# Polochon-street/bliss-rs

Measured on AMD Instinct MI355X. Metric: songs/sec (3-min 22 050 Hz f32) at 1/2/4/8 GPU; HBM GB/s vs roofline, higher is better.
Workload: dtype f32; 1 GPU; configs[1]: batch of 1024 synthetic 3969000-sample (3-min) white-noise f32 PCM buffers per GPU, full 23-feature descriptor set (FeaturesVersion 2); songs_per_gpu=1024, songs_total=1024, features=23, parallelism=single GPU

## Files before the change

### bliss-rs_amd/csrc/kernels_chroma.hip

```cpp
#include <float.h>
#include <stdlib.h>

#include <type_traits>

#include "device_utils.hpp"
#include "fft_r16.hpp"
#include "internal.hpp"

namespace bg {

typedef double double4_t __attribute__((ext_vector_type(4)));

__device__ __forceinline__ double tuning_of_slot(int slot) {
    return slot >= N_TUNING ? 0.0 : (-50.0 + (100.0 * 0.01 * (double)slot)) / 100.0;
}

__global__ __launch_bounds__(256) void chroma_bank_kernel(double* __restrict__ bank) {
#pragma clang fp contract(off)
    const int slot = blockIdx.y;
    const int k = blockIdx.x * 256 + threadIdx.x;
    if (k >= BANK_PITCH) return;
    double* out = bank + (size_t)slot * BANK_ROWS * BANK_PITCH;
    if (k >= CBINS) {
        for (int r = 0; r < BANK_ROWS; r++) out[(size_t)r * BANK_PITCH + k] = 0.0;
// ... 441 lines not shown
        const float thr = ref_floor_f32(ref);
        {
            uint32_t hits = 0;
#pragma unroll
            for (int h = 0; h < 2; h++) {
                float sb3[3], se3[3], sa3[3];
#pragma unroll
                for (int q = 0; q < 3; q++) {
                    const int c = t + 256 * (3 * h + q);
                    sb3[q] = mags[c > 0 ? c - 1 : 0];
                    se3[q] = mags[c];
                    sa3[q] = mags[c + 1];
                }
#pragma unroll
                for (int q = 0; q < 3; q++) {
                    const int j = 3 * h + q, c = t + 256 * j;
                    const uint32_t in_range = (256 * j >= PIP_LO && 256 * j + 255 <= PIP_HI) ? 1u : (uint32_t)(c >= PIP_LO) & (uint32_t)(c <= PIP_HI);
                    const uint32_t pk = in_range & (uint32_t)(sa3[q] <= se3[q]) & (uint32_t)(sb3[q] < se3[q]) & (uint32_t)(se3[q] > thr);
                    hits |= pk << j;
                }
            }
            const uint32_t mine = (uint32_t)__popc(hits);
            const uint32_t incl = wave_scan_incl_u32_dpp(mine);
            uint32_t wbase = 0;
            if (lane_id() == 63) wbase = atomicAdd(&peak_count, incl);
            uint32_t pos = (uint32_t)__builtin_amdgcn_readlane((int)wbase, 63) + incl - mine;
#pragma unroll
            for (int j = 0; j < 6; j++)
                if ((hits >> j) & 1u) peak_list[pos++] = (uint16_t)(t + 256 * j);
            TRACE(13);
            __syncthreads();
            TRACE(14);
            const uint32_t n_peaks = peak_count;
            uint32_t* __restrict__ recs = peak_rec + (sd.c_off + f) * (size_t)PIP_MAX_PER_FRAME;
            if (t == 0) peak_cnt[sd.c_off + f] = n_peaks;
            int c_next = t < n_peaks ? (int)peak_list[t] : PIP_LO;
            for (uint32_t i = t; i < n_peaks; i += 256) {
                const int c = c_next;
                const float sb = mags[c - 1], se = mags[c], sa = mags[c + 1];
                c_next = i + 256 < n_peaks ? (int)peak_list[i + 256] : PIP_LO;
                int pb;
                const uint32_t b = peak_classify(sb, se, sa, ref, c, &pb), rel = b - lbase;
                recs[i] = peak_record(b, pb, c);
                if (rel < (uint32_t)LHIST_BINS) atomicAdd(&lhist[rel], 1u);
                else atomicAdd(&hist[b], 1u);
            }
        }
        __builtin_amdgcn_s_setprio(0);
        if (has_next) {
            load_window();
#pragma unroll
            for (int n1 = 0; n1 < 16; n1++) v[n1] = v[n1] * win[n1];
        }
        TRACE(15);
        __syncthreads();
        TRACE(16);
    }
    TRACE_FLUSH();
    if (have_base) {
        const uint32_t lbase = lhist_base;
        for (int i = t; i < LHIST_BINS; i += 256) {
            const uint32_t c = lhist[i];
            if (c) atomicAdd(&hist[lbase + i], c);
        }
    }
}

void launch_stft8192(const Batch& b, const Workspace& w, const DeviceTables& t, hipStream_t st, int shape) {
    if (b.tiles_c == 0) return;
    auto k = stft8192_kernel<false, false>;
    if (shape == 1) k = stft8192_kernel<true, true>;
    else if (shape == 2) k = stft8192_kernel<true, false>;
    else if (shape == 3) k = stft8192_kernel<false, true>;
    hipLaunchKernelGGL(k, dim3((b.tiles_c + 31u) & ~31u), dim3(256), 0, st,
                       b.pcm, b.songs, b.n_songs, b.pfx_c, t.hann8192, t.tw8192, w.spec, w.frame_max, w.h1, w.peak_rec, w.peak_cnt,
                       b.tiles_c);
}

__global__ __launch_bounds__(256) void tune_select_kernel(const SongDesc* __restrict__ songs,
                                                          const uint32_t* __restrict__ h1,
                                                          TuningState* __restrict__ tuning,
                                                          uint32_t* __restrict__ cand_cursor, uint32_t cand_pool,
                                                          uint32_t first_song) {
    __shared__ uint32_t wsum[4];
    __shared__ uint32_t s_total, s_blo, s_bhi;
    const uint32_t s = blockIdx.x + first_song;
    const int tid = threadIdx.x;
    TuningState* ts = tuning + s;
    auto no_peaks = [&]() {
        if (tid == 0) {
            ts->n_peaks = 0; ts->tuning_idx = -1; ts->n_cand = 0; ts->b_lo = 1; ts->b_hi = 0; ts->below = 0;
            ts->cand_off = 0; ts->cand_cap = 0;
        }
    };
    if (!songs[s].ok) { no_peaks(); return; }
    const uint32_t* hist = h1 + (size_t)s * H1_BINS;
    constexpr int PER = H1_BINS / 256;
    uint32_t local[PER], sum = 0;
#pragma unroll
    for (int i = 0; i < PER; i++) { local[i] = hist[tid * PER + i]; sum += local[i]; }
    const uint32_t incl = wave_scan_incl_u32(sum);
    if (lane_id() == 63) wsum[wave_id()] = incl;
    __syncthreads();
    uint32_t base = 0;
    for (int w = 0; w < wave_id(); w++) base += wsum[w];
    if (tid == 255) s_total = base + incl;
    __syncthreads();
    const uint32_t total = s_total;
    uint32_t before = base + incl - sum;
    if (total == 0) { no_peaks(); return; }
    const uint32_t r_lo = (total - 1) / 2, r_hi = total - 1 - r_lo;
    if (tid == 0) { ts->n_peaks = total; ts->n_cand = 0; ts->tuning_idx = -1; }
#pragma unroll
    for (int i = 0; i < PER; i++) {
        const uint32_t c = local[i];
        if (c) {
            if (before <= r_lo && r_lo < before + c) { ts->b_lo = tid * PER + i; ts->below = before; s_blo = tid * PER + i; }
            if (before <= r_hi && r_hi < before + c) { ts->b_hi = tid * PER + i; s_bhi = tid * PER + i; }
        }
        before += c;
    }
    __syncthreads();
    const uint32_t blo = s_blo, bhi = s_bhi;
    uint32_t mine = 0;
#pragma unroll
    for (int i = 0; i < PER; i++) {
        const uint32_t bin = tid * PER + i;
        if (bin >= blo && bin <= bhi) mine += local[i];
    }
    mine = wave_sum(mine);
    if (lane_id() == 0) wsum[wave_id()] = mine;
    __syncthreads();
    if (tid == 0) {
        const uint32_t want = wsum[0] + wsum[1] + wsum[2] + wsum[3];
        const uint32_t off = atomicAdd(cand_cursor, want);
        if (off <= cand_pool && want <= cand_pool - off) {
            ts->cand_off = off;
            ts->cand_cap = want;
        } else {
            atomicSub(cand_cursor, want);
            ts->cand_off = 0;
            ts->cand_cap = 0;
        }
    }
}

void launch_tune_select(const Batch& b, const Workspace& w, hipStream_t st, const SongRange* r) {
    const uint32_t s0 = r ? r->s0 : 0, s1 = r ? r->s1 : b.n_songs;
    if (s1 <= s0) return;
    hipLaunchKernelGGL(tune_select_kernel, dim3(s1 - s0), dim3(256), 0, st, b.songs, w.h1, w.tuning, w.cand_cursor,
                       w.cand_cap, s0);
}

constexpr int P2_SLOW_CAP = 1024;
constexpr int P2_FRAMES_PER_WAVE = CH_TILE / 4;

__global__ __launch_bounds__(256) void tune_pass2_kernel(const SongDesc* __restrict__ songs, uint32_t n_songs,
                                                         const uint32_t* __restrict__ pfx_ct,
                                                         const float* __restrict__ spec,
                                                         const float* __restrict__ frame_max,
                                                         const uint32_t* __restrict__ peak_rec,
                                                         const uint32_t* __restrict__ peak_cnt,
                                                         TuningState* __restrict__ tuning,
                                                         uint32_t* __restrict__ hist100,
                                                         double* __restrict__ cand_mag,
                                                         uint8_t* __restrict__ cand_pb, uint32_t first_tile) {
    __shared__ uint32_t hist[N_TUNING];
    __shared__ uint32_t slow_list[4][P2_SLOW_CAP];
    const uint32_t bx = blockIdx.x + first_tile;
    const uint32_t s = find_segment(pfx_ct, n_songs, bx);
    const SongDesc sd = songs[s];
    const uint32_t tile = bx - pfx_ct[s];
    const int tid = threadIdx.x, lane = lane_id(), wave = wave_id();
    TuningState* ts = tuning + s;
    const uint32_t b_lo = ts->b_lo, b_hi = ts->b_hi;
    if (ts->n_peaks == 0) return;
    const uint32_t cand_off = ts->cand_off;
    const uint32_t cand_cap = ts->cand_cap;
    const bool pooled = cand_cap != 0;
    if (tid < N_TUNING) hist[tid] = 0;
    __syncthreads();
    uint32_t n_slow = 0;

    auto flush = [&]() {
        for (uint32_t i = lane; i < n_slow; i += WAVE) {
            const uint32_t e = slow_list[wave][i];
            const int c = (int)(e & 0xFFFFu);
            const uint32_t f = tile * CH_TILE + wave + 4 * (e >> 16);
            const float* row = spec + (sd.c_off + f) * (size_t)CBINS_PAD;
            const double ref = 0.1 * (double)frame_max[sd.c_off + f];
            double mag, pitch;
            if (pip_peak_core(row[c - 1], row[c], row[c + 1], ref, c, &mag, &pitch)) {
                const uint32_t b = coarse_bin(mag);
                if (b > b_hi) {
                    atomicAdd(&hist[pitch_bin(pitch)], 1u);
                } else if (b >= b_lo) {
                    const uint32_t slot = atomicAdd(&ts->n_cand, 1u);
                    if (pooled && slot < cand_cap) {
                        cand_mag[cand_off + slot] = mag;
                        cand_pb[cand_off + slot] = (uint8_t)pitch_bin(pitch);
                    }
                }
            }
        }
        __builtin_amdgcn_wave_barrier();
        n_slow = 0;
    };
    uint32_t n_rec_next = 0;
    {
        const uint32_t f0 = tile * CH_TILE + wave;
        if (f0 < sd.n_c) n_rec_next = peak_cnt[sd.c_off + f0];
    }
    for (int i = 0; i < P2_FRAMES_PER_WAVE; i++) {
        const uint32_t f = tile * CH_TILE + wave + 4 * i;
        if (f >= sd.n_c) break;
        const uint32_t n_rec = n_rec_next < (uint32_t)PIP_MAX_PER_FRAME ? n_rec_next : (uint32_t)PIP_MAX_PER_FRAME;
        if (i + 1 < P2_FRAMES_PER_WAVE && f + 4 < sd.n_c) n_rec_next = peak_cnt[sd.c_off + f + 4];
        const uint32_t* __restrict__ recs = peak_rec + (sd.c_off + f) * (size_t)PIP_MAX_PER_FRAME;
        if (n_slow + PIP_MAX_PER_FRAME > P2_SLOW_CAP) flush();
        for (uint32_t j0 = 0; j0 < n_rec; j0 += 4 * WAVE) {
            uint32_t r4[4];
#pragma unroll
            for (int u = 0; u < 4; u++) {
                const uint32_t j = j0 + WAVE * u + lane;
                r4[u] = j < n_rec ? recs[j] : 0xFFFFFFFFu;
            }
#pragma unroll
            for (int u = 0; u < 4; u++) {
                if (j0 + WAVE * u >= n_rec) break;
                const uint32_t j = j0 + WAVE * u + lane;
                bool slow = false;
                uint32_t c = 0;
                if (j < n_rec) {
                    const uint32_t r = r4[u];
                    const uint32_t b = r >> 18, pbf = (r >> 11) & 0x7Fu;
                    c = r & 0x7FFu;
                    if (b > b_hi) {
                        if (pbf) atomicAdd(&hist[pbf - 1], 1u);
                        else slow = true;
                    } else if (b >= b_lo) {
                        slow = true;
                    }
                }
                const uint64_t mask = __ballot(slow);
                if (mask) {
                    if (slow) slow_list[wave][n_slow + (uint32_t)__popcll(mask & ((1ull << lane) - 1ull))] = ((uint32_t)i << 16) | c;
                    n_slow += (uint32_t)__popcll(mask);
                }
            }
        }
    }
    __builtin_amdgcn_wave_barrier();
    flush();
    __syncthreads();
    if (tid < N_TUNING && hist[tid]) atomicAdd(&hist100[(size_t)s * N_TUNING + tid], hist[tid]);
}

void launch_tune_pass2(const Batch& b, const Workspace& w, hipStream_t st, const SongRange* r) {
    const uint32_t t0 = r ? r->ct0 : 0, t1 = r ? r->ct1 : b.tiles_ct;
    if (t1 <= t0) return;
    hipLaunchKernelGGL(tune_pass2_kernel, dim3(t1 - t0), dim3(256), 0, st, b.songs, b.n_songs, b.pfx_ct, w.spec,
                       w.frame_max, w.peak_rec, w.peak_cnt, w.tuning, w.hist100, w.cand_mag, w.cand_pb, t0);
}

template <typename ForEach>
__device__ uint64_t block_radix_select(ForEach&& for_each, uint32_t rank, uint32_t* hist, uint32_t* s_digit, uint32_t* s_rank,
                                       uint32_t* s_wave) {
    const int tid = threadIdx.x;
    uint64_t prefix = 0, mask = 0;
    for (int shift = 56; shift >= 0; shift -= 8) {
        hist[tid] = 0;
        __syncthreads();
        for_each([&](double mag, int) {
            const uint64_t k = f64_key(mag);
            const bool in = (k & mask) == prefix;
            const uint32_t d = (uint32_t)(k >> shift) & 0xFFu;
            const uint64_t m = __ballot(in);
            if (m != 0) {
                const int first = __ffsll((unsigned long long)m) - 1;
                const uint32_t d0 = (uint32_t)__shfl((int)d, first, WAVE);
                if (__ballot(in && d == d0) == m) {
                    if (lane_id() == first) atomicAdd(&hist[d0], (uint32_t)__popcll(m));
                } else if (in) {
                    atomicAdd(&hist[d], 1u);
                }
            }
        });
        __syncthreads();
        {
            const uint32_t h = hist[tid];
            const uint32_t incl = wave_scan_incl_u32(h);
            if (lane_id() == 63) s_wave[wave_id()] = incl;
            __syncthreads();
            uint32_t below = incl - h;
            for (int w = 0; w < wave_id(); w++) below += s_wave[w];
            if (h != 0 && below <= rank && rank < below + h) {
                *s_digit = (uint32_t)tid;
                *s_rank = rank - below;
            }
        }
        __syncthreads();
        prefix |= (uint64_t)(*s_digit) << shift;
        mask |= 0xFFull << shift;
        rank = *s_rank;
        __syncthreads();
    }
    return prefix;
}

__global__ __launch_bounds__(256) void tune_final_kernel(const SongDesc* __restrict__ songs,
                                                         TuningState* __restrict__ tuning,
                                                         const uint32_t* __restrict__ hist100,
                                                         const double* __restrict__ cand_mag,
                                                         const uint8_t* __restrict__ cand_pb,
                                                         const float* __restrict__ spec,
                                                         const float* __restrict__ frame_max,
                                                         const uint32_t* __restrict__ peak_rec,
                                                         const uint32_t* __restrict__ peak_cnt, uint32_t first_song) {
    __shared__ uint32_t hist[256];
    __shared__ uint32_t s_digit, s_rank, s_cnt_le, s_wave[4];
    __shared__ unsigned long long s_min_gt;
    const uint32_t s = blockIdx.x + first_song;
    const int tid = threadIdx.x;
    TuningState* ts = tuning + s;
    const SongDesc sd = songs[s];
    if (!sd.ok || ts->n_peaks == 0) return;
    const uint32_t total = ts->n_peaks, nc = ts->n_cand;
    const uint32_t r_lo = (total - 1) / 2, r_hi = total - 1 - r_lo;
    const uint32_t k_lo = r_lo - ts->below, k_hi = r_hi - ts->below;
    const uint32_t b_lo = ts->b_lo, b_hi = ts->b_hi;
    const bool pooled = ts->cand_cap != 0 && nc == ts->cand_cap;
    const double* v = cand_mag + ts->cand_off;
    const uint8_t* pb = cand_pb + ts->cand_off;

    auto for_each = [&](auto&& fn) {
        if (pooled) {
            for (uint32_t i0 = tid; i0 < nc; i0 += 8 * 256) {
                double m8[8];
                int b8[8];
#pragma unroll
                for (int u = 0; u < 8; u++) {
                    const uint32_t i = i0 + 256u * u;
                    m8[u] = i < nc ? v[i] : 0.0;
                    b8[u] = i < nc ? (int)pb[i] : 0;
                }
#pragma unroll
                for (int u = 0; u < 8; u++)
                    if (i0 + 256u * u < nc) fn(m8[u], b8[u]);
            }
        } else {
            for (uint32_t f = 0; f < sd.n_c; f++) {
                const uint32_t n_rec_raw = peak_cnt[sd.c_off + f];
                const uint32_t n_rec = n_rec_raw < (uint32_t)PIP_MAX_PER_FRAME ? n_rec_raw : (uint32_t)PIP_MAX_PER_FRAME;
                const uint32_t* __restrict__ recs = peak_rec + (sd.c_off + f) * (size_t)PIP_MAX_PER_FRAME;
                const float* __restrict__ row = spec + (sd.c_off + f) * (size_t)CBINS_PAD;
                const double ref = 0.1 * (double)frame_max[sd.c_off + f];
                for (uint32_t j = tid; j < n_rec; j += 256) {
                    const uint32_t r = recs[j], b = r >> 18;
                    if (b < b_lo || b > b_hi) continue;
                    const int c = (int)(r & 0x7FFu);
                    double mag, pitch;
                    if (pip_peak_core(row[c - 1], row[c], row[c + 1], ref, c, &mag, &pitch)) fn(mag, pitch_bin(pitch));
                }
            }
        }
    };

    const uint64_t key_lo = block_radix_select(for_each, k_lo, hist, &s_digit, &s_rank, s_wave);
    uint64_t key_hi = key_lo;
    if (k_hi != k_lo) {
        if (tid == 0) { s_cnt_le = 0; s_min_gt = ~0ull; }
        __syncthreads();
        uint32_t cnt = 0;
        unsigned long long mn = ~0ull;
        for_each([&](double mag, int) {
            const uint64_t k = f64_key(mag);
            if (k <= key_lo) cnt++;
            else if (k < mn) mn = k;
        });
        atomicAdd(&s_cnt_le, cnt);
        atomicMin(&s_min_gt, mn);
        __syncthreads();
        if (s_cnt_le <= k_hi) key_hi = s_min_gt;
    }
    double thr;
    {
#pragma clang fp contract(off)
        const double lo = key_f64(key_lo), hi = key_f64(key_hi);
        thr = lo + (hi - lo) / 2.0;
    }
    __syncthreads();
    if (tid < N_TUNING) hist[tid] = hist100[(size_t)s * N_TUNING + tid];
    __syncthreads();
    for_each([&](double mag, int bin) {
        if (mag >= thr) atomicAdd(&hist[bin], 1u);
    });
    __syncthreads();
    if (tid == 0) {
        uint32_t best = 0;
        for (uint32_t k = 1; k < N_TUNING; k++)
            if (hist[k] > hist[best]) best = k;
        ts->tuning_idx = (int32_t)best;
    }
}

void launch_tune_final(const Batch& b, const Workspace& w, hipStream_t st, const SongRange* r) {
// ... 161 lines not shown
```

### bliss-rs_amd/csrc/scheduler.hip

```cpp
#include <string.h>

#include <algorithm>
#include <chrono>
#include <condition_variable>
#include <numeric>

#include "coalescing_front.hpp"
#include "ctx.hpp"

using namespace bg;

namespace {

inline size_t align_up(size_t x, size_t a) { return (x + a - 1) / a * a; }

void fill_counts(SongDesc& d) {
    const uint64_t n = d.n;
    d.n_t = (uint32_t)((n - W512) / HOP_T + 1);
    d.n_b = (uint32_t)((n - W512) / HOP_B + 1);
    d.n_f = std::max(d.n_t, 2u * d.n_b);
    d.n_c = (uint32_t)ceilf((float)n / (float)HOP_C);
    d.n_e = (uint32_t)((n + 255) / 256);
    d.n_l = (uint32_t)((n + LOUD_W - 1) / LOUD_W);
}

size_t song_ws_bytes(const SongDesc& d) {
    if (!d.ok) return 256;
    size_t b = 0;
    b += (size_t)d.n_t * 12 + (size_t)d.n_b * 8 + (size_t)d.n_e * 8;
    b += (size_t)d.n_c * (CBINS_PAD * 4 + 4);
    b += (size_t)H1_BINS * 4 + N_TUNING * 4 + sizeof(TuningState) + sizeof(TempoState);
    b += (size_t)d.n_c * CAND_BUDGET_PER_FRAME * 9;
    b += (size_t)d.n_c * (PIP_MAX_PER_FRAME * 4 + 4);
    b += ((size_t)d.n_c / CH_TILE + 1) * 80;
    b += ((size_t)d.n_b / BT_STEP + 2) * (8 + BT_PRE_STRIDE * 4);
    return b + 4096;
}

struct Carver {
    uint8_t* base;
    size_t off = 0;
    template <typename T>
    T* take(size_t n) {
        off = align_up(off, 256);
        T* p = reinterpret_cast<T*>(base + off);
        off += n * sizeof(T);
        return p;
    }
};

struct ChunkTotals {
    uint64_t tot_t = 0, tot_b = 0, tot_c = 0, tot_e = 0;
    uint32_t max_nb = 0, max_nt = 0, max_runs = 1;
    uint32_t tiles_ct = 0;
    uint64_t cand_cap = 0;
};

Workspace carve(uint8_t* base, uint32_t ns, const ChunkTotals& t, size_t* bytes) {
    Carver m{base};
    Workspace w{};
    w.centroid = m.take<float>(t.tot_t); w.rolloff = m.take<float>(t.tot_t); w.flatness = m.take<float>(t.tot_t);
    w.flux = m.take<float>(t.tot_b); w.thresholded = m.take<float>(t.tot_b);
    w.e256 = m.take<float>(t.tot_e); w.zc256 = m.take<uint32_t>(t.tot_e);
    static_assert((size_t)(CBINS_PAD + PIP_MAX_PER_FRAME) * 4 * HOP_T >= (size_t)256 * 4 * HOP_C,
                  "the borrowed stretch must hold one 256-word entry per timbral frame: bytes per chroma frame x samples per "
                  "timbral frame >= bytes per entry x samples per chroma frame");
    w.spec = m.take<float>(t.tot_c * CBINS_PAD + 64);
    w.peak_rec = m.take<uint32_t>(t.tot_c * PIP_MAX_PER_FRAME);
    w.roll_fix_bytes = (size_t)(reinterpret_cast<uint8_t*>(w.peak_rec + t.tot_c * PIP_MAX_PER_FRAME) - reinterpret_cast<uint8_t*>(w.spec));
    w.frame_max = m.take<float>(t.tot_c);
    w.roll_fix = m.take<RollFix>(1);
    w.h1 = m.take<uint32_t>((size_t)ns * H1_BINS); w.hist100 = m.take<uint32_t>((size_t)ns * N_TUNING);
    w.tuning = m.take<TuningState>(ns);
    w.peak_cnt = m.take<uint32_t>(t.tot_c);
    w.cand_mag = m.take<double>(t.cand_cap); w.cand_pb = m.take<uint8_t>(t.cand_cap);
    w.cand_cursor = m.take<uint32_t>(4);
    w.cand_cap = (uint32_t)t.cand_cap;
    w.chroma_part = m.take<double>((size_t)t.tiles_ct * 10 + 16);
    w.tempo = m.take<TempoState>(ns);
    w.run_bpm = m.take<float>((size_t)ns * t.max_runs); w.run_cnt = m.take<uint32_t>((size_t)ns * t.max_runs);
    w.runs_pitch = t.max_runs;
    w.bt_pre = m.take<float>((size_t)(t.tot_b / BT_STEP + ns + 1) * BT_PRE_STRIDE);
    w.summary = m.take<float>((size_t)ns * 16);
    *bytes = m.off + 4096;
    return w;
}

int ensure_mask_stream(blissgpu_ctx* c, int cus) {
    cus = std::max(1, std::min(cus, c->n_cus));
    if (c->mask_stream && c->mask_cus == cus) return BLISSGPU_OK;
    if (c->mask_stream) { (void)hipStreamSynchronize(c->mask_stream); (void)hipStreamDestroy(c->mask_stream); c->mask_stream = nullptr; }
    std::vector<uint32_t> mask((size_t)(c->n_cus + 31) / 32, 0u);
    for (int i = 0; i < cus; i++) mask[(size_t)i / 32] |= 1u << (i % 32);
    HIP_TRY(hipExtStreamCreateWithCUMask(&c->mask_stream, (uint32_t)mask.size(), mask.data()));
    c->mask_cus = cus;
    return BLISSGPU_OK;
}

int ensure_slot_events(ChunkSlot& s) {
    if (s.ev_free) return BLISSGPU_OK;
    hipEvent_t* evs[] = {&s.ev_start, &s.ev_fork, &s.ev_stft, &s.ev_sel, &s.ev_tune, &s.ev_sum, &s.ev_chroma, &s.ev_desc, &s.ev_free, &s.ev_acf, &s.ev_beat};
    for (hipEvent_t* e : evs) HIP_TRY(hipEventCreateWithFlags(e, hipEventDisableTiming));
    for (hipEvent_t& e : s.ev_piece) HIP_TRY(hipEventCreateWithFlags(&e, hipEventDisableTiming));
    return BLISSGPU_OK;
}

int chunk_front(blissgpu_ctx* c, ChunkSlot& slot, const float* d_pcm, SongDesc* songs, uint32_t ns, bool only_chunk) {
    int rc = ensure_slot_events(slot);
    if (rc) return rc;
    std::vector<uint32_t> pfx_f(ns + 1, 0), pfx_c(ns + 1, 0), pfx_ct(ns + 1, 0), pfx_cw(ns + 1, 0);
    ChunkTotals t;
    for (uint32_t i = 0; i < ns; i++) {
        SongDesc& d = songs[i];
        d.t_off = t.tot_t; d.b_off = t.tot_b; d.c_off = t.tot_c; d.e_off = t.tot_e;
        if (d.ok) {
            t.tot_t += d.n_t; t.tot_b += d.n_b; t.tot_c += d.n_c; t.tot_e += d.n_e;
            t.max_nb = std::max(t.max_nb, d.n_b);
            t.max_nt = std::max(t.max_nt, d.n_t);
            t.max_runs = std::max(t.max_runs, d.n_b / BT_STEP + 1);
        }
        pfx_f[i + 1] = pfx_f[i] + (d.ok ? (d.n_f + F512_TILE - 1) / F512_TILE : 0);
        pfx_c[i + 1] = pfx_c[i] + (d.ok ? 4 * ((d.n_c + 4 * STFT_TILE - 1) / (4 * STFT_TILE)) : 0);
        pfx_ct[i + 1] = pfx_ct[i] + (d.ok ? (d.n_c + CH_TILE - 1) / CH_TILE : 0);
        pfx_cw[i + 1] = pfx_cw[i] + (d.ok ? (d.n_c + 4 * CH_TILE - 1) / (4 * CH_TILE) : 0);
    }
    t.tiles_ct = pfx_ct[ns];
    t.cand_cap = std::min<uint64_t>(t.tot_c * (uint64_t)c->cand_budget, 0xFFFFFF00ull) + 64;

    const size_t desc_bytes = align_up(ns * sizeof(SongDesc), 256) + 4 * align_up((ns + 1) * 4, 256) + 256;
    size_t need = 0;
    (void)carve(nullptr, ns, t, &need);
    if ((rc = slot.desc.ensure(desc_bytes))) return rc;
    if ((rc = slot.slab.ensure(need))) return rc;
    if (slot.used) HIP_TRY(hipEventSynchronize(slot.ev_desc));
    if ((rc = slot.h_desc.ensure(desc_bytes))) return rc;

    hipStream_t st = c->stream, sb = c->serial ? c->stream : c->aux_stream, sc = c->serial ? c->stream : c->chr_stream;
    const bool multi = !c->serial;
    if (slot.used && multi) HIP_TRY(hipStreamWaitEvent(st, slot.ev_free, 0));

    uint8_t* h = slot.h_desc.p;
    size_t o = 0;
    const size_t o_songs = o; memcpy(h + o, songs, ns * sizeof(SongDesc)); o = align_up(o + ns * sizeof(SongDesc), 256);
    const size_t o_f = o; memcpy(h + o, pfx_f.data(), (ns + 1) * 4); o = align_up(o + (ns + 1) * 4, 256);
    const size_t o_c = o; memcpy(h + o, pfx_c.data(), (ns + 1) * 4); o = align_up(o + (ns + 1) * 4, 256);
    const size_t o_ct = o; memcpy(h + o, pfx_ct.data(), (ns + 1) * 4); o = align_up(o + (ns + 1) * 4, 256);
    const size_t o_cw = o; memcpy(h + o, pfx_cw.data(), (ns + 1) * 4); o = align_up(o + (ns + 1) * 4, 256);
    HIP_TRY(hipMemcpyAsync(slot.desc.p, h, o, hipMemcpyHostToDevice, st));
    slot.used = true;

    Batch& b = slot.batch;
    b = Batch{};
    b.pcm = d_pcm;
    b.songs = reinterpret_cast<const SongDesc*>(slot.desc.p + o_songs);
    b.n_songs = ns;
    b.pfx_f = reinterpret_cast<const uint32_t*>(slot.desc.p + o_f);
    b.pfx_c = reinterpret_cast<const uint32_t*>(slot.desc.p + o_c);
    b.pfx_ct = reinterpret_cast<const uint32_t*>(slot.desc.p + o_ct);
    b.pfx_cw = reinterpret_cast<const uint32_t*>(slot.desc.p + o_cw);
    b.tiles_f = pfx_f[ns]; b.tiles_c = pfx_c[ns]; b.tiles_ct = pfx_ct[ns]; b.tiles_cw = pfx_cw[ns];
    b.total_b = t.tot_b; b.max_nb = t.max_nb; b.max_nt = t.max_nt;

    size_t used_bytes = 0;
    slot.ws = carve(slot.slab.p, ns, t, &used_bytes);
    slot.ws.dbg_chroma = nullptr;
    slot.ws.dbg_interval = nullptr;
    if (c->debug_chroma) {
        if ((rc = c->dbg_chroma.ensure((size_t)t.tot_c * 12 + 12))) return rc;
        if ((rc = c->dbg_interval.ensure((size_t)ns * 10))) return rc;
        slot.ws.dbg_chroma = c->dbg_chroma.p;
        slot.ws.dbg_interval = c->dbg_interval.p;
    }
    const Workspace& w = slot.ws;
    c->last_ws = w;
    c->last_songs.assign(songs, songs + ns);
    {
        RollFix rf{};
        if ((uint64_t)w.roll_fix_bytes / (256 * 4) < t.tot_t)
            return fail(BLISSGPU_ERR_INVALID, "chunk_front", "internal: the borrowed stretch cannot hold one exact-rolloff entry per timbral frame");
        rf.cap = (uint32_t)t.tot_t;
        rf.mags = w.spec;
        memcpy(h + o, &rf, sizeof(rf));
        HIP_TRY(hipMemcpyAsync(w.roll_fix, h + o, sizeof(rf), hipMemcpyHostToDevice, st));
    }
    HIP_TRY(hipEventRecord(slot.ev_desc, st));

    HIP_TRY(hipMemsetAsync(w.h1, 0, (size_t)ns * H1_BINS * 4, st));
    HIP_TRY(hipMemsetAsync(w.hist100, 0, (size_t)ns * N_TUNING * 4, st));
    HIP_TRY(hipMemsetAsync(w.cand_cursor, 0, 16, st));
    { Prof p(c, K_FFT512); launch_fft512(b, w, c->tables, st, c->rolloff_exact_all, c->flux_order); }
    { Prof p(c, K_ROLLFIX); launch_rolloff_fix(b, w, t.tot_t, st); }
    if (multi) {
        HIP_TRY(hipEventRecord(slot.ev_fork, st));
        HIP_TRY(hipStreamWaitEvent(sb, slot.ev_fork, 0));
    }
    { Prof p(c, K_ONSET, sb); launch_onset(b, w, sb); }
    { Prof p(c, K_SUMMARY, sb); launch_summary(b, w, sb); }
    slot.beat_masked = multi && c->tail_mode >= 2;
    if (slot.beat_masked) {
        if ((rc = ensure_mask_stream(c, c->tail_mode))) return rc;
        { Prof p(c, K_BEAT, sb); launch_beat_acf(b, w, c->tables, sb); }
        HIP_TRY(hipEventRecord(slot.ev_acf, sb));
        HIP_TRY(hipStreamWaitEvent(c->mask_stream, slot.ev_acf, 0));
        { Prof p(c, K_BEAT, c->mask_stream); launch_beat_track(b, w, c->tables, c->mask_stream); }
        HIP_TRY(hipEventRecord(slot.ev_beat, c->mask_stream));
    }
    const bool acf_early = multi && c->tail_mode == -2;
    if (acf_early) { Prof p(c, K_BEAT, sb); launch_beat_acf(b, w, c->tables, sb); }
    const bool beat_last = multi && c->tail_mode == -3;
    const bool beat_late = !slot.beat_masked && !beat_last && (c->tail_mode == 1 || acf_early || (c->tail_mode < 0 && only_chunk));
    if (!beat_late && !slot.beat_masked && !beat_last) { Prof p(c, K_BEAT, sb); launch_beat(b, w, c->tables, sb); }
    { Prof p(c, K_STFT8192); launch_stft8192(b, w, c->tables, st, c->stft_shape); }
    if (multi) {
        HIP_TRY(hipEventRecord(slot.ev_stft, st));
        HIP_TRY(hipStreamWaitEvent(sc, slot.ev_stft, 0));
    }
    slot.pieces = 0;
    if (multi && only_chunk && c->tail_split > 1 && ns >= 2) {
        const int want = std::min<int>(std::min<int>(c->tail_split, ChunkSlot::MAX_PIECES), (int)ns);
        uint32_t s0 = 0;
        for (int k = 0; k < want && s0 < ns; k++) {
            uint32_t s1 = s0 + 1;
            const uint64_t goal = (uint64_t)pfx_ct[ns] * (uint64_t)(k + 1) / (uint64_t)want;
            while (s1 < ns && (k == want - 1 || pfx_ct[s1] < goal)) s1++;
            slot.piece[slot.pieces++] = SongRange{s0, s1, pfx_ct[s0], pfx_ct[s1], pfx_cw[s0], pfx_cw[s1]};
            s0 = s1;
        }
        if (slot.pieces < 2) slot.pieces = 0;
    }
    if (slot.pieces) {
        for (int k = 0; k < slot.pieces; k++) {
            { Prof p(c, K_TUNE_SELECT, sc); launch_tune_select(b, w, sc, &slot.piece[k]); }
            if (k == 1 && beat_late) {
                HIP_TRY(hipEventRecord(slot.ev_sel, sc));
                HIP_TRY(hipStreamWaitEvent(sb, slot.ev_sel, 0));
                Prof p(c, K_BEAT, sb);
                if (acf_early) launch_beat_track(b, w, c->tables, sb); else launch_beat(b, w, c->tables, sb);
            }
            { Prof p(c, K_TUNE_PASS2, sc); launch_tune_pass2(b, w, sc, &slot.piece[k]); }
            { Prof p(c, K_TUNE_FINAL, sc); launch_tune_final(b, w, sc, &slot.piece[k]); }
            HIP_TRY(hipEventRecord(slot.ev_piece[k], sc));
        }
        if (beat_last) {
            HIP_TRY(hipStreamWaitEvent(sb, slot.ev_piece[slot.pieces - 1], 0));
            Prof p(c, K_BEAT, sb);
            launch_beat(b, w, c->tables, sb);
        }
        HIP_TRY(hipGetLastError());
        slot.back_pending = true;
        return BLISSGPU_OK;
    }
    { Prof p(c, K_TUNE_SELECT, sc); launch_tune_select(b, w, sc); }
    if (beat_late) {
        if (multi) {
            HIP_TRY(hipEventRecord(slot.ev_sel, sc));
            HIP_TRY(hipStreamWaitEvent(sb, slot.ev_sel, 0));
        }
        Prof p(c, K_BEAT, sb);
        if (acf_early) launch_beat_track(b, w, c->tables, sb); else launch_beat(b, w, c->tables, sb);
    }
    { Prof p(c, K_TUNE_PASS2, sc); launch_tune_pass2(b, w, sc); }
    { Prof p(c, K_TUNE_FINAL, sc); launch_tune_final(b, w, sc); }
    if (multi) HIP_TRY(hipEventRecord(slot.ev_tune, sc));
    if (beat_last) {
        HIP_TRY(hipStreamWaitEvent(sb, slot.ev_tune, 0));
        Prof p(c, K_BEAT, sb);
        launch_beat(b, w, c->tables, sb);
    }
    HIP_TRY(hipGetLastError());
    slot.back_pending = true;
    return BLISSGPU_OK;
}

int chunk_back(blissgpu_ctx* c, ChunkSlot& slot, uint32_t features_version, float* d_out, int32_t* d_status) {
    if (!slot.back_pending) return BLISSGPU_OK;
    slot.back_pending = false;
    hipStream_t st = c->stream, sb = c->serial ? c->stream : c->aux_stream;
    const bool multi = !c->serial;
    if (slot.pieces) {
        for (int k = 0; k < slot.pieces; k++) {
            HIP_TRY(hipStreamWaitEvent(st, slot.ev_piece[k], 0));
            Prof p(c, K_CHROMA);
            launch_chroma(slot.batch, slot.ws, c->tables, st, &slot.piece[k]);
        }
    } else {
        if (multi) HIP_TRY(hipStreamWaitEvent(st, slot.ev_tune, 0));
        Prof p(c, K_CHROMA);
        launch_chroma(slot.batch, slot.ws, c->tables, st);
    }
    if (multi) {
        HIP_TRY(hipEventRecord(slot.ev_chroma, st));
        HIP_TRY(hipStreamWaitEvent(sb, slot.ev_chroma, 0));
        if (slot.beat_masked) HIP_TRY(hipStreamWaitEvent(sb, slot.ev_beat, 0));
    }
    { Prof p(c, K_FINALIZE, sb); launch_finalize(slot.batch, slot.ws, features_version, d_out, d_status, c->dbg_tuning.p, c->dbg_nbpms.p, sb); }
    if (multi) HIP_TRY(hipEventRecord(slot.ev_free, sb));
    HIP_TRY(hipGetLastError());
    return BLISSGPU_OK;
}

}

namespace bg {

void scheduler_release(blissgpu_ctx* c) {
    for (ChunkSlot& s : c->slot) {
        s.slab.release(); s.desc.release(); s.h_desc.release();
        hipEvent_t evs[] = {s.ev_start, s.ev_fork, s.ev_stft, s.ev_sel, s.ev_tune, s.ev_sum, s.ev_chroma, s.ev_desc, s.ev_free, s.ev_acf, s.ev_beat};
        for (hipEvent_t e : evs)
            if (e) (void)hipEventDestroy(e);
        for (hipEvent_t e : s.ev_piece)
            if (e) (void)hipEventDestroy(e);
        s = ChunkSlot{};
    }
    HostFeed& f = c->feed;
    f.ring.reset();
    for (hipStream_t& ls : f.lane_stream)
        if (ls) { (void)hipStreamSynchronize(ls); (void)hipStreamDestroy(ls); ls = nullptr; }
    for (auto& row : f.ev_lane)
        for (hipEvent_t& ev : row)
            if (ev) { (void)hipEventDestroy(ev); ev = nullptr; }
    for (auto& kv : c->swr_banks)
        if (kv.second.d_bank) (void)hipFree(kv.second.d_bank);
    c->swr_banks.clear();
    c->swr_bytes = 0;
    for (hipStream_t& cs : f.copy_stream)
        if (cs) { (void)hipStreamSynchronize(cs); (void)hipStreamDestroy(cs); cs = nullptr; }
    for (int b = 0; b < N_FEED_BUFFERS; b++) {
        f.pcm[b].release(); f.raw[b].release(); f.out[b].release();
        for (hipEvent_t& ev : f.ev_copied[b])
            if (ev) { (void)hipEventDestroy(ev); ev = nullptr; }
        if (f.ev_done[b]) (void)hipEventDestroy(f.ev_done[b]);
        f.ev_done[b] = nullptr;
    }
}

#ifndef FEED_GROUP_MIB
// ... 656 lines not shown
```

Measured before the change: 27690 songs/sec.

## Software-pipeline tuning pass-2 record loads and batch slow-path flush gathers

Restructures tune_pass2_kernel so that each wave prefetches the next frame's peak records while it classifies the current one, and reads all per-frame counts with a single lane-parallel load plus readlane. Slow-path entries are compacted with a DPP wave scan over per-lane bitmasks instead of one ballot per word. The flush loop now issues four gathers of spectrum and frame_max per lane before it computes anything. Separately, the slow list grows to 2000 entries with launch bounds set for five workgroups per CU. The host also folds the RollFix record into the single descriptor memcpy, dropping one small H2D copy. The costs are more registers and LDS per workgroup, and a workspace pointer that now lives in the descriptor buffer.

Measured after the change: 27770 songs/sec, median of 6. Within noise of the previous version (+0.3%).

```diff
diff --git a/bliss-rs_amd/csrc/kernels_chroma.hip b/bliss-rs_amd/csrc/kernels_chroma.hip
--- a/bliss-rs_amd/csrc/kernels_chroma.hip
+++ b/bliss-rs_amd/csrc/kernels_chroma.hip
@@ -617,21 +617,26 @@
                        w.cand_cap, s0);
 }
 
-constexpr int P2_SLOW_CAP = 1024;
+constexpr int P2_SLOW_CAP = 2000;
 constexpr int P2_FRAMES_PER_WAVE = CH_TILE / 4;
-
-__global__ __launch_bounds__(256) void tune_pass2_kernel(const SongDesc* __restrict__ songs, uint32_t n_songs,
-                                                         const uint32_t* __restrict__ pfx_ct,
-                                                         const float* __restrict__ spec,
-                                                         const float* __restrict__ frame_max,
-                                                         const uint32_t* __restrict__ peak_rec,
-                                                         const uint32_t* __restrict__ peak_cnt,
-                                                         TuningState* __restrict__ tuning,
-                                                         uint32_t* __restrict__ hist100,
-                                                         double* __restrict__ cand_mag,
-                                                         uint8_t* __restrict__ cand_pb, uint32_t first_tile) {
+constexpr int P2_FLUSH = 4;
+constexpr int P2_WORDS = (PIP_MAX_PER_FRAME + WAVE - 1) / WAVE;
+static_assert(P2_WORDS <= 16 && P2_FRAMES_PER_WAVE <= WAVE, "a lane keeps one bit per record and one frame count per wave slot");
+
+__global__ __launch_bounds__(256, 5) void tune_pass2_kernel(const SongDesc* __restrict__ songs, uint32_t n_songs,
+                                                            const uint32_t* __restrict__ pfx_ct,
+                                                            const float* __restrict__ spec,
+                                                            const float* __restrict__ frame_max,
+                                                            const uint32_t* __restrict__ peak_rec,
+                                                            const uint32_t* __restrict__ peak_cnt,
+                                                            TuningState* __restrict__ tuning,
+                                                            uint32_t* __restrict__ hist100,
+                                                            double* __restrict__ cand_mag,
+                                                            uint8_t* __restrict__ cand_pb, uint32_t first_tile) {
     __shared__ uint32_t hist[N_TUNING];
     __shared__ uint32_t slow_list[4][P2_SLOW_CAP];
+    static_assert(5 * sizeof(uint32_t) * (4 * P2_SLOW_CAP + N_TUNING) <= 160 * 1024 && 6 * sizeof(uint32_t) * (4 * P2_SLOW_CAP + N_TUNING) > 160 * 1024,
+                  "exactly five workgroups fit a CU's 160 KiB of LDS");
     const uint32_t bx = blockIdx.x + first_tile;
     const uint32_t s = find_segment(pfx_ct, n_songs, bx);
     const SongDesc sd = songs[s];
@@ -648,22 +653,34 @@
     uint32_t n_slow = 0;
 
     auto flush = [&]() {
-        for (uint32_t i = lane; i < n_slow; i += WAVE) {
-            const uint32_t e = slow_list[wave][i];
-            const int c = (int)(e & 0xFFFFu);
-            const uint32_t f = tile * CH_TILE + wave + 4 * (e >> 16);
-            const float* row = spec + (sd.c_off + f) * (size_t)CBINS_PAD;
-            const double ref = 0.1 * (double)frame_max[sd.c_off + f];
-            double mag, pitch;
-            if (pip_peak_core(row[c - 1], row[c], row[c + 1], ref, c, &mag, &pitch)) {
-                const uint32_t b = coarse_bin(mag);
-                if (b > b_hi) {
-                    atomicAdd(&hist[pitch_bin(pitch)], 1u);
-                } else if (b >= b_lo) {
-                    const uint32_t slot = atomicAdd(&ts->n_cand, 1u);
-                    if (pooled && slot < cand_cap) {
-                        cand_mag[cand_off + slot] = mag;
-                        cand_pb[cand_off + slot] = (uint8_t)pitch_bin(pitch);
+        for (uint32_t i0 = 0; i0 < n_slow; i0 += P2_FLUSH * WAVE) {
+            int cc[P2_FLUSH];
+            float sb[P2_FLUSH], se[P2_FLUSH], sa[P2_FLUSH], fm[P2_FLUSH];
+#pragma unroll
+            for (int u = 0; u < P2_FLUSH; u++) {
+                const uint32_t i = i0 + (uint32_t)(WAVE * u + lane);
+                const uint32_t e = slow_list[wave][i < n_slow ? i : 0u];
+                const size_t fr = sd.c_off + tile * CH_TILE + wave + 4 * (e >> 16);
+                const int c = (int)(e & 0xFFFFu);
+                const float* row = spec + fr * (size_t)CBINS_PAD;
+                cc[u] = c;
+                sb[u] = row[c - 1]; se[u] = row[c]; sa[u] = row[c + 1];
+                fm[u] = frame_max[fr];
+            }
+#pragma unroll
+            for (int u = 0; u < P2_FLUSH; u++) {
+                const double ref = 0.1 * (double)fm[u];
+                double mag, pitch;
+                if (i0 + (uint32_t)(WAVE * u + lane) < n_slow && pip_peak_core(sb[u], se[u], sa[u], ref, cc[u], &mag, &pitch)) {
+                    const uint32_t b = coarse_bin(mag);
+                    if (b > b_hi) {
+                        atomicAdd(&hist[pitch_bin(pitch)], 1u);
+                    } else if (b >= b_lo) {
+                        const uint32_t slot = atomicAdd(&ts->n_cand, 1u);
+                        if (pooled && slot < cand_cap) {
+                            cand_mag[cand_off + slot] = mag;
+                            cand_pb[cand_off + slot] = (uint8_t)pitch_bin(pitch);
+                        }
                     }
                 }
             }
@@ -671,52 +688,61 @@
         __builtin_amdgcn_wave_barrier();
         n_slow = 0;
     };
-    uint32_t n_rec_next = 0;
+    uint32_t cnt_l = 0;
     {
-        const uint32_t f0 = tile * CH_TILE + wave;
-        if (f0 < sd.n_c) n_rec_next = peak_cnt[sd.c_off + f0];
-    }
-    for (int i = 0; i < P2_FRAMES_PER_WAVE; i++) {
-        const uint32_t f = tile * CH_TILE + wave + 4 * i;
-        if (f >= sd.n_c) break;
-        const uint32_t n_rec = n_rec_next < (uint32_t)PIP_MAX_PER_FRAME ? n_rec_next : (uint32_t)PIP_MAX_PER_FRAME;
-        if (i + 1 < P2_FRAMES_PER_WAVE && f + 4 < sd.n_c) n_rec_next = peak_cnt[sd.c_off + f + 4];
+        const uint32_t f = tile * CH_TILE + wave + 4 * (uint32_t)lane;
+        if (lane < P2_FRAMES_PER_WAVE && f < sd.n_c) {
+            const uint32_t n = peak_cnt[sd.c_off + f];
+            cnt_l = n < (uint32_t)PIP_MAX_PER_FRAME ? n : (uint32_t)PIP_MAX_PER_FRAME;
+        }
+    }
+    auto request = [&](int i, uint32_t (&r)[P2_WORDS]) {
+        const uint32_t f = tile * CH_TILE + wave + 4 * (uint32_t)i;
+        const uint32_t n = i < P2_FRAMES_PER_WAVE ? (uint32_t)__builtin_amdgcn_readlane((int)cnt_l, i) : 0u;
         const uint32_t* __restrict__ recs = peak_rec + (sd.c_off + f) * (size_t)PIP_MAX_PER_FRAME;
-        if (n_slow + PIP_MAX_PER_FRAME > P2_SLOW_CAP) flush();
-        for (uint32_t j0 = 0; j0 < n_rec; j0 += 4 * WAVE) {
-            uint32_t r4[4];
-#pragma unroll
-            for (int u = 0; u < 4; u++) {
-                const uint32_t j = j0 + WAVE * u + lane;
-                r4[u] = j < n_rec ? recs[j] : 0xFFFFFFFFu;
-            }
-#pragma unroll
-            for (int u = 0; u < 4; u++) {
-                if (j0 + WAVE * u >= n_rec) break;
-                const uint32_t j = j0 + WAVE * u + lane;
-                bool slow = false;
-                uint32_t c = 0;
-                if (j < n_rec) {
-                    const uint32_t r = r4[u];
-                    const uint32_t b = r >> 18, pbf = (r >> 11) & 0x7Fu;
-                    c = r & 0x7FFu;
-                    if (b > b_hi) {
-                        if (pbf) atomicAdd(&hist[pbf - 1], 1u);
-                        else slow = true;
-                    } else if (b >= b_lo) {
-                        slow = true;
-                    }
-                }
-                const uint64_t mask = __ballot(slow);
-                if (mask) {
-                    if (slow) slow_list[wave][n_slow + (uint32_t)__popcll(mask & ((1ull << lane) - 1ull))] = ((uint32_t)i << 16) | c;
-                    n_slow += (uint32_t)__popcll(mask);
-                }
-            }
-        }
-    }
-    __builtin_amdgcn_wave_barrier();
-    flush();
+#pragma unroll
+        for (int u = 0; u < P2_WORDS; u++) {
+            const uint32_t j = (uint32_t)(WAVE * u + lane);
+            r[u] = (uint32_t)(WAVE * u) < n ? recs[j < n ? j : 0u] : 0u;
+        }
+    };
+    auto file = [&](int i, const uint32_t (&r)[P2_WORDS]) {
+        const uint32_t n_rec = (uint32_t)__builtin_amdgcn_readlane((int)cnt_l, i);
+        uint32_t slow_bits = 0;
+#pragma unroll
+        for (int u = 0; u < P2_WORDS; u++) {
+            if ((uint32_t)(WAVE * u) >= n_rec) break;
+            const uint32_t b = r[u] >> 18, pbf = (r[u] >> 11) & 0x7Fu;
+            const bool valid = (uint32_t)(WAVE * u + lane) < n_rec;
+            const bool fast = valid & (b > b_hi) & (pbf != 0u);
+            if (fast) atomicAdd(&hist[pbf - 1], 1u);
+            const bool slow = valid & (b >= b_lo) & !fast;
+            slow_bits |= slow ? 1u << u : 0u;
+        }
+        if (__ballot(slow_bits != 0u)) {
+            const uint32_t mine = (uint32_t)__popc(slow_bits);
+            const uint32_t incl = wave_scan_incl_u32_dpp(mine);
+            uint32_t pos = n_slow + incl - mine;
+            n_slow += (uint32_t)__builtin_amdgcn_readlane((int)incl, WAVE - 1);
+#pragma unroll
+            for (int u = 0; u < P2_WORDS; u++)
+                if ((slow_bits >> u) & 1u) slow_list[wave][pos++] = ((uint32_t)i << 16) | (r[u] & 0x7FFu);
+        }
+    };
+    uint32_t cur[P2_WORDS], nxt[P2_WORDS];
+    request(0, nxt);
+    for (int i = 0;; i++) {
+        const bool done = i == P2_FRAMES_PER_WAVE || tile * CH_TILE + wave + 4 * (uint32_t)i >= sd.n_c;
+        if (done || n_slow + PIP_MAX_PER_FRAME > P2_SLOW_CAP) {
+            __builtin_amdgcn_wave_barrier();
+            flush();
+        }
+        if (done) break;
+#pragma unroll
+        for (int u = 0; u < P2_WORDS; u++) cur[u] = nxt[u];
+        request(i + 1, nxt);
+        file(i, cur);
+    }
     __syncthreads();
     if (tid < N_TUNING && hist[tid]) atomicAdd(&hist100[(size_t)s * N_TUNING + tid], hist[tid]);
 }
diff --git a/bliss-rs_amd/csrc/scheduler.hip b/bliss-rs_amd/csrc/scheduler.hip
--- a/bliss-rs_amd/csrc/scheduler.hip
+++ b/bliss-rs_amd/csrc/scheduler.hip
@@ -69,7 +69,7 @@
     w.peak_rec = m.take<uint32_t>(t.tot_c * PIP_MAX_PER_FRAME);
     w.roll_fix_bytes = (size_t)(reinterpret_cast<uint8_t*>(w.peak_rec + t.tot_c * PIP_MAX_PER_FRAME) - reinterpret_cast<uint8_t*>(w.spec));
     w.frame_max = m.take<float>(t.tot_c);
-    w.roll_fix = m.take<RollFix>(1);
+    w.roll_fix = nullptr;
     w.h1 = m.take<uint32_t>((size_t)ns * H1_BINS); w.hist100 = m.take<uint32_t>((size_t)ns * N_TUNING);
     w.tuning = m.take<TuningState>(ns);
     w.peak_cnt = m.take<uint32_t>(t.tot_c);
@@ -146,6 +146,20 @@
     const size_t o_c = o; memcpy(h + o, pfx_c.data(), (ns + 1) * 4); o = align_up(o + (ns + 1) * 4, 256);
     const size_t o_ct = o; memcpy(h + o, pfx_ct.data(), (ns + 1) * 4); o = align_up(o + (ns + 1) * 4, 256);
     const size_t o_cw = o; memcpy(h + o, pfx_cw.data(), (ns + 1) * 4); o = align_up(o + (ns + 1) * 4, 256);
+    size_t used_bytes = 0;
+    slot.ws = carve(slot.slab.p, ns, t, &used_bytes);
+    const size_t o_rf = o;
+    {
+        static_assert(sizeof(RollFix) <= 256, "the descriptor block reserves 256 bytes for the record");
+        RollFix rf{};
+        if ((uint64_t)slot.ws.roll_fix_bytes / (256 * 4) < t.tot_t)
+            return fail(BLISSGPU_ERR_INVALID, "chunk_front", "internal: the borrowed stretch cannot hold one exact-rolloff entry per timbral frame");
+        rf.cap = (uint32_t)t.tot_t;
+        rf.mags = slot.ws.spec;
+        memcpy(h + o, &rf, sizeof(rf));
+        o += sizeof(rf);
+        slot.ws.roll_fix = reinterpret_cast<RollFix*>(slot.desc.p + o_rf);
+    }
     HIP_TRY(hipMemcpyAsync(slot.desc.p, h, o, hipMemcpyHostToDevice, st));
     slot.used = true;
 
@@ -161,8 +175,6 @@
     b.tiles_f = pfx_f[ns]; b.tiles_c = pfx_c[ns]; b.tiles_ct = pfx_ct[ns]; b.tiles_cw = pfx_cw[ns];
     b.total_b = t.tot_b; b.max_nb = t.max_nb; b.max_nt = t.max_nt;
 
-    size_t used_bytes = 0;
-    slot.ws = carve(slot.slab.p, ns, t, &used_bytes);
     slot.ws.dbg_chroma = nullptr;
     slot.ws.dbg_interval = nullptr;
     if (c->debug_chroma) {
@@ -174,15 +186,6 @@
     const Workspace& w = slot.ws;
     c->last_ws = w;
     c->last_songs.assign(songs, songs + ns);
-    {
-        RollFix rf{};
-        if ((uint64_t)w.roll_fix_bytes / (256 * 4) < t.tot_t)
-            return fail(BLISSGPU_ERR_INVALID, "chunk_front", "internal: the borrowed stretch cannot hold one exact-rolloff entry per timbral frame");
-        rf.cap = (uint32_t)t.tot_t;
-        rf.mags = w.spec;
-        memcpy(h + o, &rf, sizeof(rf));
-        HIP_TRY(hipMemcpyAsync(w.roll_fix, h + o, sizeof(rf), hipMemcpyHostToDevice, st));
-    }
     HIP_TRY(hipEventRecord(slot.ev_desc, st));
 
     HIP_TRY(hipMemsetAsync(w.h1, 0, (size_t)ns * H1_BINS * 4, st));
```
